# lbrndnr/LBAudioDetective

Measured on AMD Instinct MI355X. Metric: audio_seconds_fingerprinted_per_sec, higher is better.
Workload: dtype f32; 1 GPU; configs[1]: 100k synthetic 1 s @44.1 kHz mono clips, 1024-pt FFT, stride 64, fingerprint-only, input resident in HBM; one step = 13 passes over the batch; clips_per_gpu=100000, samples_per_clip=44100, window=1024, stride=64, bands=32, subfingerprints_per_clip=5, kernel_variant=0, parallelism=clips sharded x1, no collective

## Files before the change

include/lbaudiodetective.h:

```cpp
#ifndef LBAUDIODETECTIVE_H
#define LBAUDIODETECTIVE_H

#include <stddef.h>
#include <stdint.h>

#ifdef __cplusplus
extern "C" {
#endif

#if !defined(__MACTYPES__) && !defined(LBAD_HAVE_MACTYPES)
typedef uint32_t UInt32;
typedef int32_t SInt32;
typedef uint64_t UInt64;
typedef int64_t SInt64;
typedef float Float32;
typedef double Float64;
typedef unsigned char Boolean;
typedef SInt32 OSStatus;
enum { noErr = 0 };
#endif

#if !defined(__CoreAudioTypes_h__) && !defined(LBAD_HAVE_COREAUDIOTYPES)
typedef struct AudioStreamBasicDescription {
    Float64 mSampleRate;
// ... 123 lines not shown

OSStatus LBAudioDetectiveProcessPCM(LBAudioDetectiveRef inDetective, const Float32* inSamples,
                                    UInt64 inNumberOfSamples, LBAudioDetectiveFingerprintRef* outFingerprint);
OSStatus LBAudioDetectiveComparePCM(LBAudioDetectiveRef inDetective, const Float32* inSamples1, UInt64 inCount1,
                                    const Float32* inSamples2, UInt64 inCount2, UInt32 inComparisonRange,
                                    Float32* outMatch);

#define LBAD_PACKED_WORDS 8
#define LBAD_PACKED_BYTES 32
#define LBAD_MAX_SUBFINGERPRINT_LENGTH 256

OSStatus LBAudioDetectiveFingerprintClipsDevice(LBAudioDetectiveRef inDetective, const Float32* inClips,
                                                UInt64 inNumberOfClips, UInt64 inSamplesPerClip,
                                                void* outPacked, void* inStream);
OSStatus LBAudioDetectiveFingerprintClipsDeviceFormat(LBAudioDetectiveRef inDetective, const void* inClips,
                                                      UInt32 inSampleFormat, UInt64 inNumberOfClips,
                                                      UInt64 inSamplesPerClip, void* outPacked, void* inStream);
OSStatus LBAudioDetectiveFingerprintClips(LBAudioDetectiveRef inDetective, const Float32* inClips,
                                          UInt64 inNumberOfClips, UInt64 inSamplesPerClip, Boolean* outBooleans);
OSStatus LBAudioDetectiveFingerprintClipsFormat(LBAudioDetectiveRef inDetective, const void* inClips,
                                                UInt32 inSampleFormat, UInt64 inNumberOfClips,
                                                UInt64 inSamplesPerClip, Boolean* outBooleans);
OSStatus LBAudioDetectiveSetKernelVariant(LBAudioDetectiveRef inDetective, UInt32 inVariant);
OSStatus LBAudioDetectiveSetKernelTuning(LBAudioDetectiveRef inDetective, UInt32 inWavesPerWorkgroup,
                                         UInt32 inTwiddleCache);
OSStatus LBAudioDetectiveSetScratchLimit(LBAudioDetectiveRef inDetective, UInt64 inBytes);
OSStatus LBAudioDetectiveSetStageTiming(LBAudioDetectiveRef inDetective, UInt32 inEnabled);
OSStatus LBAudioDetectiveGetStageTimes(LBAudioDetectiveRef inDetective, Float32* outStage1Ms, Float32* outStage2Ms,
                                       UInt32* outLaunches);
OSStatus LBAudioDetectiveFingerprintClipsDeviceTaps(LBAudioDetectiveRef inDetective, const Float32* inClips,
                                                    UInt64 inNumberOfClips, UInt64 inSamplesPerClip,
                                                    void* outPacked, Float32* outFramesRaw, Float32* outFramesHaar,
                                                    void* inStream);
OSStatus LBAudioDetectiveFingerprintClipsDeviceTapsFormat(LBAudioDetectiveRef inDetective, const void* inClips,
                                                          UInt32 inSampleFormat, UInt64 inNumberOfClips,
                                                          UInt64 inSamplesPerClip, void* outPacked, Float32* outFramesRaw,
                                                          Float32* outFramesHaar, void* inStream);
OSStatus LBAudioDetectiveDebugStage1Choice(Float64 inSampleRate, UInt32 inWindowSize, UInt32 inAnalysisStride,
                                           UInt32 inNumberOfPitchSteps, UInt32 inSubfingerprintLength, UInt32 inKernelVariant,
                                           UInt32 inWavesPerWorkgroup, UInt32 inTwiddleCache, UInt32 inSampleFormat,
                                           UInt64 inNumberOfClips, UInt64 inSamplesPerClip, UInt32 inClipAddressMod8,
                                           UInt32 inRawTap, UInt32 inFileTail, UInt32* outWords, UInt32 inCapacity);

typedef struct LBAudioDetectiveStream* LBAudioDetectiveStreamRef;
LBAudioDetectiveStreamRef LBAudioDetectiveStreamNew(LBAudioDetectiveRef inDetective);
void LBAudioDetectiveStreamDispose(LBAudioDetectiveStreamRef inStream);
// ... 260 lines not shown
```

lbaudiodetective_amd/_native.py:

```python
from __future__ import annotations

import ctypes as C
import os
import subprocess

_HERE = os.path.dirname(os.path.abspath(__file__))
CSRC = os.path.join(_HERE, "csrc")
LIB_PATH = os.path.abspath(os.environ["LBAD_LIB"]) if os.environ.get("LBAD_LIB") else os.path.join(_HERE, "lib", "liblbaudiodetective.so")
HEADER = os.path.join(os.path.dirname(_HERE), "include", "lbaudiodetective.h")

UInt32, SInt32, UInt64, SInt64 = C.c_uint32, C.c_int32, C.c_uint64, C.c_int64
Float32, Float64, Boolean, OSStatus = C.c_float, C.c_double, C.c_ubyte, C.c_int32
Ref = C.c_void_p

PACKED_WORDS = 8
PACKED_BYTES = 32
SHARD_KEYS = 4096
ROWS_PER_FRAME = 128


class AudioStreamBasicDescription(C.Structure):
    _fields_ = [
        ("mSampleRate", Float64), ("mFormatID", UInt32), ("mFormatFlags", UInt32),
        ("mBytesPerPacket", UInt32), ("mFramesPerPacket", UInt32), ("mBytesPerFrame", UInt32),
# ... 67 lines not shown
    "LBAudioDetectiveSetResamplerMode": (OSStatus, [Ref, UInt32]),
    "LBAudioDetectiveReadAudioURLWithResampler": (OSStatus, [C.c_char_p, Float64, UInt32, _P(_P(Float32)), _P(UInt64),
                                                            _P(Float64)]),
    "LBAudioDetectiveProcessFileStream": (OSStatus, [Ref, C.c_void_p, UInt64, UInt64, UInt32, _P(Ref)]),
    "LBAudioDetectiveReadAudioURL": (OSStatus, [C.c_char_p, Float64, _P(_P(Float32)), _P(UInt64), _P(Float64)]),
    "LBAudioDetectiveFreeSamples": (None, [_P(Float32)]),
    "LBAudioDetectiveGetSubfingerprintCount": (UInt64, [Ref, UInt64]),
    "LBAudioDetectiveProcessPCM": (OSStatus, [Ref, C.c_void_p, UInt64, _P(Ref)]),
    "LBAudioDetectiveComparePCM": (OSStatus, [Ref, C.c_void_p, UInt64, C.c_void_p, UInt64, UInt32, _P(Float32)]),
    "LBAudioDetectiveFingerprintClipsDevice": (OSStatus, [Ref, C.c_void_p, UInt64, UInt64, C.c_void_p, C.c_void_p]),
    "LBAudioDetectiveFingerprintClipsDeviceFormat": (OSStatus, [Ref, C.c_void_p, UInt32, UInt64, UInt64, C.c_void_p, C.c_void_p]),
    "LBAudioDetectiveSetFilePipeline": (OSStatus, [Ref, UInt32]),
    "LBAudioDetectiveGetCompactLayout": (OSStatus, [Ref, _P(UInt32), _P(UInt32)]),
    "LBAudioDetectiveGetCompactBands": (OSStatus, [Ref, _P(UInt32), _P(UInt32)]),
    "LBAudioDetectiveCompactFramesToSubfingerprintsDevice": (OSStatus, [Ref, C.c_void_p, UInt64, C.c_void_p, C.c_void_p, C.c_void_p]),
    "LBAudioDetectiveFramesToSubfingerprintsDevice": (OSStatus, [Ref, C.c_void_p, UInt64, C.c_void_p, C.c_void_p, C.c_void_p]),
    "LBAudioDetectiveStreamNew": (Ref, [Ref]),
    "LBAudioDetectiveStreamDispose": (None, [Ref]),
    "LBAudioDetectiveStreamPush": (OSStatus, [Ref, C.c_void_p, UInt64, _P(UInt32)]),
    "LBAudioDetectiveStreamCopyFingerprint": (Ref, [Ref]),
    "LBAudioDetectiveFingerprintClips": (OSStatus, [Ref, C.c_void_p, UInt64, UInt64, C.c_void_p]),
    "LBAudioDetectiveFingerprintClipsFormat": (OSStatus, [Ref, C.c_void_p, UInt32, UInt64, UInt64, C.c_void_p]),
    "LBAudioDetectiveSetKernelVariant": (OSStatus, [Ref, UInt32]),
    "LBAudioDetectiveSetScratchLimit": (OSStatus, [Ref, UInt64]),
    "LBAudioDetectiveSetStageTiming": (OSStatus, [Ref, UInt32]),
    "LBAudioDetectiveGetStageTimes": (OSStatus, [Ref, _P(Float32), _P(Float32), _P(UInt32)]),
    "LBAudioDetectiveFingerprintClipsDeviceTapsFormat": (OSStatus, [Ref, C.c_void_p, UInt32, UInt64, UInt64, C.c_void_p, C.c_void_p,
                                                                    C.c_void_p, C.c_void_p]),
    "LBAudioDetectiveDebugStage1Choice": (OSStatus, [Float64, UInt32, UInt32, UInt32, UInt32, UInt32, UInt32, UInt32, UInt32, UInt64,
                                                     UInt64, UInt32, UInt32, UInt32, _P(UInt32), UInt32]),
    "LBAudioDetectiveFingerprintClipsDeviceTaps": (OSStatus, [Ref, C.c_void_p, UInt64, UInt64, C.c_void_p, C.c_void_p,
                                                              C.c_void_p, C.c_void_p]),
    "LBAudioDetectivePackSubfingerprint": (None, [C.c_void_p, UInt32, C.c_void_p]),
    "LBAudioDetectiveUnpackSubfingerprint": (None, [C.c_void_p, UInt32, C.c_void_p]),
    "LBAudioDetectiveCorpusNew": (Ref, [UInt32, UInt32, UInt64]),
    "LBAudioDetectiveCorpusNewRagged": (Ref, [UInt32, UInt64, UInt64]),
    "LBAudioDetectiveCorpusAppendRaggedPackedDevice": (OSStatus, [Ref, C.c_void_p, C.c_void_p, UInt64, C.c_void_p]),
    "LBAudioDetectiveCorpusGetSubfingerprintTotal": (UInt64, [Ref]),
    "LBAudioDetectiveSynthRaggedCorpusDevice": (OSStatus, [UInt32, UInt64, UInt64, C.c_void_p, UInt64, UInt32, C.c_void_p,
                                                           C.c_void_p]),
    "LBAudioDetectiveCorpusQuerySharded": (OSStatus, [Ref, Ref, UInt32, UInt64, C.c_void_p, C.c_void_p, _P(SInt64), _P(Float32)]),
    "LBAudioDetectiveCorpusQueryBatchSharded": (OSStatus, [Ref, _P(Ref), UInt32, UInt32, UInt64, C.c_void_p, C.c_void_p,
                                                           _P(SInt64), _P(Float32)]),
    "LBAudioDetectiveCorpusQueryBatchShardedWith": (OSStatus, [Ref, _P(Ref), UInt32, UInt32, UInt64, C.c_void_p, C.c_void_p,
                                                               C.c_void_p, _P(SInt64), _P(Float32)]),
    "LBAudioDetectiveSetExchangeTimeout": (None, [UInt32]),
# ... 145 lines not shown
```

lbaudiodetective_amd/api.py:

```python
from __future__ import annotations

import collections
import ctypes as C

import numpy as np

from . import _native as N

noErr = 0


class LBAudioDetectiveError(RuntimeError):
    def __init__(self, status: int, what: str):
        self.status = status
        code = status & 0xFFFFFFFF
        four = bytes([(code >> s) & 0xFF for s in (24, 16, 8, 0)])
        tag = f"'{four.decode()}'" if all(32 <= b < 127 for b in four) else str(status)
        super().__init__(f"{what}: OSStatus {tag}")


def _check(status: int, what: str):
    if status != noErr:
        raise LBAudioDetectiveError(status, what)

# ... 216 lines not shown

    def set_window_size_status(self, v: int) -> int:
        return self._L.LBAudioDetectiveSetWindowSize(self._ref, int(v))

    def configure(self, sample_rate=None, window=None, stride=None, bands=None, subfp_len=None) -> "Detective":
        if sample_rate is not None:
            self.processing_sample_rate = sample_rate
        if window is not None:
            self.window_size = window
        if stride is not None:
            self.analysis_stride = stride
        if bands is not None:
            self.number_of_pitch_steps = bands
        if subfp_len is not None:
            self.subfingerprint_length = subfp_len
        return self

    def set_file_pipeline(self, enabled: bool):
        _check(self._L.LBAudioDetectiveSetFilePipeline(self._ref, 1 if enabled else 0), "SetFilePipeline")
        return self

    def set_kernel_variant(self, variant: int):
        _check(self._L.LBAudioDetectiveSetKernelVariant(self._ref, variant), "SetKernelVariant")

    def set_scratch_limit(self, n_bytes: int):
        _check(self._L.LBAudioDetectiveSetScratchLimit(self._ref, n_bytes), "SetScratchLimit")

    def set_stage_timing(self, enabled: bool):
        _check(self._L.LBAudioDetectiveSetStageTiming(self._ref, int(enabled)), "SetStageTiming")

    def stage_times(self):
        a, b, n = N.Float32(0), N.Float32(0), N.UInt32(0)
        _check(self._L.LBAudioDetectiveGetStageTimes(self._ref, C.byref(a), C.byref(b), C.byref(n)), "GetStageTimes")
        return float(a.value), float(b.value), int(n.value)

    def subfingerprint_count(self, n_samples: int) -> int:
        return int(self._L.LBAudioDetectiveGetSubfingerprintCount(self._ref, n_samples))

    def set_kernel_tuning(self, waves_per_workgroup: int = 0, twiddle_cache: bool = True):
        _check(self._L.LBAudioDetectiveSetKernelTuning(self._ref, waves_per_workgroup, int(twiddle_cache)), "SetKernelTuning")
        return self

    def set_file_hop_mode(self, mode: int):
        _check(self._L.LBAudioDetectiveSetFileHopMode(self._ref, mode), "SetFileHopMode")
        return self

# ... 1064 lines not shown
```

lbaudiodetective_amd/csrc/api_detective.cpp:

```cpp
#include "internal.hpp"
#include "const_div.hpp"

#include <new>
#include "audiofile.hpp"

#include <cmath>
#include <cstdlib>
#include <cstring>

namespace lbad {

uint64_t subfingerprint_count(uint64_t n_samples, uint32_t window, uint32_t stride) {
    if (stride == 0 || n_samples < window) return 0;
    return ((n_samples - window) / stride) / kRowsPerFrame;
}

static bool valid_window(uint32_t w) { return w >= kMinWindow && w <= kMaxWindow && (w & (w - 1)) == 0; }

static void free_plan(Plan& p) { p = Plan(); }

static void plan_kernels_host(Plan& p) {
    p.pruned_ok = rows_pruned_supported(p);
    p.full_ok = rows_full_supported(p);
    p.stream_ok = rows_stream_supported(p);
    p.stream2_ok = rows_stream2_supported(p);
}

static OSStatus plan_kernels_device(Plan& p) {
    if (p.pruned_ok && !p.d_bin_const) {
        std::vector<float> bc;
        rows_pruned_constants(bc);
        OSStatus st = p.d_bin_const.reserve(bc.size());
        if (st != noErr) return st;
        LBAD_HIP(hipMemcpy(p.d_bin_const, bc.data(), bc.size() * sizeof(float), hipMemcpyHostToDevice));
    }
    return p.full_ok || p.stream_ok || p.stream2_ok ? p.d_claim.reserve(8) : noErr;
}

OSStatus plan_host(Plan& p, double rate, uint32_t window, uint32_t stride, uint32_t bands, uint32_t subfp_len) {
    if (!valid_window(window) || stride == 0 || bands == 0 || bands > kMaxBands || !(rate > 0.0) || subfp_len == 0 ||
        subfp_len > LBAD_MAX_SUBFINGERPRINT_LENGTH || subfp_len > kRowsPerFrame * bands)
        return kLBAudioDetectiveArgumentInvalid;
    p.sample_rate = rate;
    p.window = window;
    p.stride = stride;
// ... 41 lines not shown
    LBAD_HIP(hipMemcpy(p.d_tw, re.data(), half * sizeof(float), hipMemcpyHostToDevice));
    LBAD_HIP(hipMemcpy(p.d_tw + half, im.data(), half * sizeof(float), hipMemcpyHostToDevice));
    std::vector<uint32_t> tbl(11 * (size_t)p.bands);
    for (uint32_t b = 0; b < p.bands; ++b) {
        tbl[b] = p.table.lo[b];
        tbl[p.bands + b] = p.table.hi[b];
        const float div = (float)(p.table.indices[b + 1] - p.table.indices[b]);
        std::memcpy(&tbl[2 * p.bands + b], &div, 4);
        tbl[3 * p.bands + b] = p.bands;
        tbl[4 * p.bands + b] = b;
        uint32_t mult = 0, off = 0xFFFFFFFFu;
        if (p.sparse.ok) {
            const uint32_t pos = b >= 16 ? p.sparse.pos_right[b - 16] : (b == p.sparse.left ? p.sparse.pos_left : 0xFFu);
            if (pos != 0xFFu) { mult = p.sparse.n_stored; off = pos; }
        }
        tbl[5 * p.bands + b] = mult;
        tbl[6 * p.bands + b] = off;
        tbl[7 * p.bands + b] = p.table.term_at[b];
        const float rcp = 1.0f / div;
        std::memcpy(&tbl[9 * p.bands + b], &rcp, 4);
        tbl[10 * p.bands + b] = band_div_proven(div) ? 1u : 0u;
    }
    tbl[8 * (size_t)p.bands] = p.table.term_end;
    st = p.d_bands.reserve(tbl.size());
    if (st != noErr) return st;
    LBAD_HIP(hipMemcpy(p.d_bands, tbl.data(), tbl.size() * sizeof(uint32_t), hipMemcpyHostToDevice));
    st = plan_kernels_device(p);
    if (st != noErr) return st;
    p.valid = true;
    return noErr;
}

static hipError_t apply_file_tail(const Plan& p, const FileTail& t, const void* d_pcm, uint64_t rows_total, float* frames,
                                  hipStream_t stream) {
    if (t.mode == 3) return launch_empty_rows_batch(p, t.d_files, t.n_files, t.max_rows, frames, stream);
    const uint64_t rows = t.rows ? t.rows : rows_total;
    if (t.first_short >= rows) return hipSuccess;
    float* file_frames = frames + t.row_begin * p.bands;
    if (t.mode == 1)
        return launch_empty_rows(p, file_frames + t.first_short * p.bands, rows - t.first_short, stream);
    if (t.mode == 2)
        return launch_file_tail(p, static_cast<const float*>(d_pcm) + t.pcm_begin, t.n_client, p.stride, t.first_short,
                                (uint32_t)(rows - t.first_short), t.d_tbl, file_frames, stream);
    return hipSuccess;
}

// ... 80 lines not shown
    }
    w[7] = ch.compact ? 1u : 0u;
    w[8] = ch.stage2_select32 ? (ch.compact ? 2u : 1u) : 0u;
    w[11] = (uint32_t)ch.per;
}

OSStatus fingerprint_clips_device(LBAudioDetective* d, const void* d_pcm_raw, uint32_t fmt, uint64_t n_clips,
                                  uint64_t spc, uint32_t* d_packed, float* d_raw, float* d_haar, hipStream_t stream,
                                  const FileTail* tail, size_t n_tails) {
    if (fmt > 2) return kLBAudioDetectiveArgumentInvalid;
    if (tail && (n_clips != 1 || fmt != 0)) return kLBAudioDetectiveArgumentInvalid;
    LBAD_LOCK(d);
    const size_t elem = fmt == 1 ? 2 : 4;
    const char* d_pcm = static_cast<const char*>(d_pcm_raw);
    OSStatus st = ensure_plan(d);
    if (st != noErr) return st;
    const Plan& p = d->plan;
    Stage1Call call;
    call.variant = d->variant; call.fmt = fmt; call.n_clips = n_clips; call.spc = spc;
    call.ptr_mod8 = (uint32_t)(reinterpret_cast<uintptr_t>(d_pcm_raw) % 8);
    call.raw_tap = d_raw != nullptr; call.tail = tail != nullptr;
    const Stage1Choice ch = stage1_choose(p, call);
    if (ch.status != noErr || !ch.launches) return ch.status;
    const uint64_t per = ch.per;
    StreamOrder order{d, stream};
    LBAD_HIP(order.begin());
    const bool compact = ch.compact;
    auto stage1 = [&](const void* pcm_in, uint64_t nc, float* frames_out) -> hipError_t {
        switch (ch.family) {
            case Stage1Family::Pruned:
                return launch_rows_pruned(p, p.d_bin_const, pcm_in, fmt, nc, spc, (uint32_t)per, frames_out, stream, compact);
            case Stage1Family::Stream2: return launch_rows_stream2(p, pcm_in, fmt, nc, spc, (uint32_t)per, frames_out, stream);
            case Stage1Family::Full: return launch_rows_full(p, pcm_in, fmt, nc, spc, (uint32_t)per, frames_out, stream);
            case Stage1Family::Stream: return launch_rows_stream(p, pcm_in, fmt, nc, spc, (uint32_t)per, frames_out, stream);
            case Stage1Family::Generic: break;
        }
        return launch_fft_bands(p, pcm_in, fmt, nc, spc, (uint32_t)per, frames_out, stream);
    };
    auto stage2 = [&](float* frames_in, uint64_t nf, uint32_t* packed_out, float* haar_out) -> hipError_t {
        if (compact && haar_out) {
            hipError_t e = hipMemsetAsync(haar_out, 0, nf * kRowsPerFrame * p.bands * sizeof(float), stream);
            if (e != hipSuccess) return e;
        }
        return ch.stage2_select32 ? launch_haar_select32(p, frames_in, nf, packed_out, haar_out, stream, compact)
                                  : launch_haar_select(p, frames_in, nf, packed_out, haar_out, stream);
    };
    const uint64_t frame_floats = (uint64_t)kRowsPerFrame * p.bands;
    if (d_raw) {
        LBAD_HIP(stage1(d_pcm, n_clips, d_raw));
        for (size_t t = 0; tail && t < n_tails; ++t) LBAD_HIP(apply_file_tail(p, tail[t], d_pcm, per * kRowsPerFrame, d_raw, stream));
        LBAD_HIP(stage2(d_raw, n_clips * per, d_packed, d_haar));
        return noErr;
    }
    uint64_t chunk = (d->scratch_limit / sizeof(float)) / (per * frame_floats);
// ... 225 lines not shown
    LBAD_LOCK(d);
    d->subfp_len = inSubfingerprintLength;
    return noErr;
}
OSStatus LBAudioDetectiveSetWindowSize(LBAudioDetectiveRef d, UInt32 inWindowSize) {
    LBAD_LOCK(d);
    if (!lbad::valid_window(inWindowSize)) return kLBAudioDetectiveArgumentInvalid;
    d->window = inWindowSize;
    return noErr;
}
OSStatus LBAudioDetectiveSetAnalysisStride(LBAudioDetectiveRef d, UInt32 inAnalysisStride) {
    LBAD_LOCK(d);
    d->stride = inAnalysisStride;
    return noErr;
}

OSStatus LBAudioDetectiveSetKernelVariant(LBAudioDetectiveRef d, UInt32 inVariant) {
    LBAD_LOCK(d);
    if (inVariant > 4) return kLBAudioDetectiveArgumentInvalid;
    d->variant = inVariant;
    return noErr;
}

OSStatus LBAudioDetectiveSetKernelTuning(LBAudioDetectiveRef d, UInt32 inWavesPerWorkgroup, UInt32 inTwiddleCache) {
    LBAD_LOCK(d);
    if (!d || inWavesPerWorkgroup > 16) return kLBAudioDetectiveArgumentInvalid;
    d->tune_waves = inWavesPerWorkgroup;
    d->tune_cache = inTwiddleCache != 0;
    return noErr;
}

OSStatus LBAudioDetectiveSetScratchLimit(LBAudioDetectiveRef d, UInt64 inBytes) {
    LBAD_LOCK(d);
    if (!d || inBytes == 0) return kLBAudioDetectiveArgumentInvalid;
    d->scratch_limit = inBytes;
    return noErr;
}

OSStatus LBAudioDetectiveSetStageTiming(LBAudioDetectiveRef d, UInt32 inEnabled) {
    LBAD_LOCK(d);
    if (!d) return kLBAudioDetectiveArgumentInvalid;
    d->timing = inEnabled != 0;
    d->ev_used = 0;
    return noErr;
}

// ... 511 lines not shown
```

lbaudiodetective_amd/csrc/internal.hpp:

```cpp
#pragma once

#include <hip/hip_runtime.h>

#include <algorithm>
#include <cstdint>
#include <cstdio>
#include <new>
#include <stdexcept>
#include <map>
#include <mutex>
#include <vector>

#include "../../include/lbaudiodetective.h"
#include "buffers.hpp"

namespace lbad {

constexpr uint32_t kRowsPerFrame = 128;
constexpr uint32_t kPackedWords = LBAD_PACKED_WORDS;
constexpr uint32_t kMaxBands = 64;
constexpr uint32_t kSparseFrameDwMax = 128 * 17;
constexpr uint32_t kMinWindow = 16;
constexpr uint32_t kMaxWindow = 8192;

// ... 23 lines not shown
    std::vector<uint32_t> lo, hi;
    uint32_t kmin = 0, kmax = 0;
    std::vector<uint32_t> term_at;
    uint32_t term_end = 0;
    bool ordered = true;
    uint64_t unread_terms16 = 0;
};

void make_band_table(double sample_rate, uint32_t window, uint32_t bands, BandTable& out);
void make_band_bounds(double sample_rate, uint32_t window, uint32_t n_frames, const BandTable& table, uint32_t* lo,
                      uint32_t* hi);
void make_twiddles(uint32_t W, std::vector<float>& re, std::vector<float>& im);

struct Plan {
    double sample_rate = 0;
    uint32_t window = 0, stride = 0, bands = 0, subfp_len = 0;
    uint32_t log2w = 0;
    uint32_t keep = 0;
    BandTable table;
    DeviceBuffer<float> d_tw;
    DeviceBuffer<uint32_t> d_bands;
    DeviceBuffer<float> d_bin_const;
    bool pruned_ok = false;
    bool full_ok = false;
    bool stream_ok = false;
    bool stream2_ok = false;
    DeviceBuffer<uint32_t> d_claim;
    struct Sparse {
        bool ok = false;
        uint32_t left = 32;
        uint32_t n_cols = 0;
        uint8_t cols[32] = {};
        uint32_t n_stored = 0;
        uint8_t stored[17] = {};
        uint8_t pos_right[16];
        uint8_t pos_left = 0xFF;
        uint32_t frame_dw() const { return 128u * n_stored; }
    } sparse;
    uint32_t tune_waves = 0;
    bool tune_cache = true;
    bool valid = false;
};

struct FileDesc;
struct FileTail {
    uint32_t mode = 0;
    const FileDesc* d_files = nullptr;
    uint32_t n_files = 0;
    uint64_t max_rows = 0;
    uint64_t first_short = 0;
    uint64_t n_client = 0;
    const uint32_t* d_tbl = nullptr;
    uint64_t row_begin = 0;
    uint64_t rows = 0;
    uint64_t pcm_begin = 0;
};

hipError_t launch_fft_bands(const Plan& plan, const void* d_pcm, uint32_t fmt, uint64_t n_clips,
                            uint64_t samples_per_clip, uint32_t frames_per_clip, float* d_frames, hipStream_t stream);
hipError_t launch_haar_select(const Plan& plan, float* d_frames, uint64_t n_frames, uint32_t* d_packed,
                              float* d_haar_out, hipStream_t stream);
bool rows_pruned_supported(const Plan& plan);
void rows_pruned_constants(std::vector<float>& out);
hipError_t launch_rows_pruned(const Plan& plan, const float* d_bin_const, const void* d_pcm, uint32_t fmt,
                              uint64_t n_clips, uint64_t samples_per_clip, uint32_t frames_per_clip, float* d_frames,
                              hipStream_t stream, bool compact = false);

bool rows_full_supported(const Plan& plan);
bool rows_full_supported_fmt(const Plan& plan, uint32_t fmt);
hipError_t launch_rows_full(const Plan& plan, const void* d_pcm, uint32_t fmt, uint64_t n_clips,
                            uint64_t samples_per_clip, uint32_t frames_per_clip, float* d_frames, hipStream_t stream);

bool rows_stream_supported(const Plan& plan);
hipError_t launch_rows_stream(const Plan& plan, const void* d_pcm, uint32_t fmt, uint64_t n_clips,
                              uint64_t samples_per_clip, uint32_t frames_per_clip, float* d_frames, hipStream_t stream);

bool rows_stream2_supported(const Plan& plan);
hipError_t launch_rows_stream2(const Plan& plan, const void* d_pcm, uint32_t fmt, uint64_t n_clips,
                               uint64_t samples_per_clip, uint32_t frames_per_clip, float* d_frames, hipStream_t stream);

bool haar_select32_supported(const Plan& plan);
hipError_t launch_haar_select32(const Plan& plan, const float* d_frames, uint64_t n_frames, uint32_t* d_packed,
                                float* d_haar_out, hipStream_t stream, bool compact = false);
void plan_sparse(Plan& plan);

enum class Stage1Family : uint32_t { Generic = 0, Pruned = 1, Stream2 = 2, Full = 3, Stream = 4 };
struct FftBandsInstance {
    uint32_t log2w = 0, wpb = 0;
    bool cached = false;
// ... 353 lines not shown

}

struct LBAudioDetectiveFingerprint {
    uint32_t length = 0;
    uint32_t count = 0;
    std::vector<Boolean> data;
};

struct LBAudioDetectiveFrame {
    uint32_t max_rows = 0;
    uint32_t n_rows = 0;
    uint32_t row_length = 0;
    std::vector<std::vector<Float32>> rows;
};

struct LBAudioDetective {
    AudioStreamBasicDescription format;
    uint32_t subfp_len;
    uint32_t window;
    uint32_t stride;
    uint32_t bands;
    uint32_t variant = 0;
    uint32_t tune_waves = 0;
    bool tune_cache = true;
    uint32_t hop_mode = 1;
    uint32_t tail_mode = 1;
    uint32_t resampler = 0;
    lbad::Plan plan;
    lbad::DeviceBuffer<float> d_frames;
    uint64_t scratch_limit = 512ull << 20;
    lbad::DeviceBuffer<void> d_io_pcm;
    lbad::DeviceBuffer<uint32_t> d_io_packed;
    lbad::PinnedBuffer<void> h_io;
    hipStream_t io_stream = nullptr;
    lbad::DeviceBuffer<uint8_t> d_rs_bytes[2];
    hipStream_t up_stream = nullptr;
    hipEvent_t up_done[2] = {nullptr, nullptr};
    hipEvent_t bytes_free[2] = {nullptr, nullptr};
    hipEvent_t packed_done[2] = {nullptr, nullptr};
    lbad::DeviceBuffer<float> d_rs_in;
    lbad::DeviceBuffer<float> d_rs_out;
    lbad::DeviceBuffer<double> d_rs_table[2];
    std::vector<lbad::DevPhase> d_phases;
    lbad::DeviceBuffer<lbad::FileDesc> d_rs_desc;
    lbad::DeviceBuffer<uint32_t> d_rs_tail;
// ... 82 lines not shown
```

lbaudiodetective_amd/csrc/k_rows_pruned.hip:

```cpp
#include "internal.hpp"
#include "const_div.hpp"
#include "fft64_lane.hpp"

namespace lbad {
namespace {

constexpr int kW = 1024;
constexpr int kStride = 64;
constexpr int kBands = 32;
constexpr int kBins = 22;
constexpr int kRows = 43;
constexpr int kRowsA = 22;
constexpr int kRowDw = 20;
constexpr int kWinDw = 464;
constexpr int kWaves = 4;
constexpr int kThreads = kWaves * 64;
constexpr int kUnitWindows = 32;
constexpr int kSpan = (kUnitWindows - 1) * kStride + kW;
constexpr int kSpanDw = kSpan + 16 * (kSpan >> 6);
constexpr int kTDw = kWaves * 8 * kWinDw;
constexpr int kBinConst = 14;
constexpr int kConstStride = 20;
constexpr int kConstDw = kBins * kConstStride;
constexpr int kClaimOffset = 312;
// ... 319 lines not shown
#ifdef LBAD_EXP_TIMELINE
        STAMP(6);
        if (lane == 0) {
            float* o = frames + ((unit >> 2) * 128 + quarter * kUnitWindows + 8 * wave) * kBands;
            for (int i = 1; i < 7; ++i) o[i - 1] = (float)(ts[i] - ts[i - 1]);
            o[6] = (float)(ts[0] & 0xFFFFFF);
            o[7] = (float)__builtin_amdgcn_s_getreg(((16 - 1) << 11) | 4);
            o[8] = (float)(ts[0] >> 24 & 0xFFFFFF);
            o[9] = (float)(__builtin_amdgcn_s_memrealtime() - rt0);
        }
#endif
        if (next >= xcd_end) break;
        unit = next;
    }
#ifndef LBAD_EXP_TIMELINE
    if (out_ptr) {
#pragma unroll
        for (int q = 0; q < 4; ++q) out_ptr[q * 2 * b_mult] = out[q];
    }
#endif
    if (claimer) claims_done(claim_ctr);
}

}

bool rows_pruned_supported(const Plan& p) {
    if (p.window != (uint32_t)kW || p.stride != (uint32_t)kStride || p.bands != (uint32_t)kBands) return false;
    if (p.table.kmax > (uint32_t)kBins) return false;
    std::vector<float> re, im;
    make_twiddles(kW, re, im);
    for (int t = 0; t < 32; ++t)
        if (re[16 * t] != kTw64Re[t] || im[16 * t] != kTw64Im[t]) return false;
    return true;
}

void rows_pruned_constants(std::vector<float>& out) {
    std::vector<float> re, im;
    make_twiddles(kW, re, im);
    out.assign((size_t)kClaimOffset + kClaimWords, 0.0f);
    for (int k = 0; k < kBins; ++k) {
        float* c = &out[(size_t)k * kBinConst];
        c[0] = re[8 * k]; c[1] = im[8 * k];
        c[2] = re[4 * k]; c[3] = im[4 * k];
        c[4] = re[2 * k]; c[5] = im[2 * k];
        if (k > 0) {
            c[6] = -re[8 * (64 - k)];   c[7] = -im[8 * (64 - k)];
            c[8] = -re[4 * (128 - k)];  c[9] = -im[4 * (128 - k)];
            c[10] = -re[2 * (256 - k)]; c[11] = -im[2 * (256 - k)];
            c[12] = re[k]; c[13] = im[k];
        }
    }
}

template <int FMT>
static hipError_t launch_rows_fmt(const Plan& plan, const float* d_bin_const, const void* d_pcm, uint64_t n_frames,
                                  uint64_t samples_per_clip, uint32_t frames_per_clip, float* d_frames,
                                  hipStream_t stream, bool compact) {
    static PerDevice attr;
    if (attr.changed(kLdsBytes)) {
        hipError_t e = hipFuncSetAttribute(reinterpret_cast<const void*>(frame_rows_pruned_kernel<FMT>),
                                           hipFuncAttributeMaxDynamicSharedMemorySize, kLdsBytes);
        if (e != hipSuccess) return e;
    }
    const uint64_t n_units = n_frames * 4, units_per_xcd = 4 * ((n_frames + 7) / 8);
    const int n_cu = device_cu_count();
    uint64_t wg_per_xcd = ((uint64_t)n_cu * kWgPerCu + 7) / 8;
    if (wg_per_xcd > units_per_xcd / 4) wg_per_xcd = units_per_xcd / 4;
    uint32_t* claim = reinterpret_cast<uint32_t*>(const_cast<float*>(d_bin_const)) + kClaimOffset;
    hipLaunchKernelGGL(frame_rows_pruned_kernel<FMT>, dim3((uint32_t)(wg_per_xcd * 8)), dim3(kThreads), kLdsBytes,
                       stream, d_pcm, samples_per_clip, frames_per_clip, n_units, units_per_xcd, d_bin_const,
                       plan.d_bands, claim, d_frames, compact ? plan.sparse.frame_dw() : 128u * kBands, compact ? 5u : 3u);
    return hipGetLastError();
}

hipError_t launch_rows_pruned(const Plan& plan, const float* d_bin_const, const void* d_pcm, uint32_t fmt,
                              uint64_t n_clips, uint64_t samples_per_clip, uint32_t frames_per_clip, float* d_frames,
                              hipStream_t stream, bool compact) {
    if (compact && !plan.sparse.ok) return hipErrorInvalidValue;
    const uint64_t n_frames = n_clips * frames_per_clip;
    if (n_frames == 0) return hipSuccess;
    if (n_frames > 0x7fffffffull) return hipErrorInvalidValue;
    if (n_frames * 4 + 8 > 0x7fffffffull) return hipErrorInvalidValue;
    switch (fmt) {
        case 0: return launch_rows_fmt<0>(plan, d_bin_const, d_pcm, n_frames, samples_per_clip, frames_per_clip, d_frames, stream, compact);
        case 1: return launch_rows_fmt<1>(plan, d_bin_const, d_pcm, n_frames, samples_per_clip, frames_per_clip, d_frames, stream, compact);
        case 2: return launch_rows_fmt<2>(plan, d_bin_const, d_pcm, n_frames, samples_per_clip, frames_per_clip, d_frames, stream, compact);
        default: return hipErrorInvalidValue;
    }
}

}
```

Before: 5.509 million audio-s/s.

## Add lane-mapped band-sum pruned FFT kernel, selected by default

```diff
diff --git a/include/lbaudiodetective.h b/include/lbaudiodetective.h
--- a/include/lbaudiodetective.h
+++ b/include/lbaudiodetective.h
@@ -169,6 +169,8 @@
                                                 UInt32 inSampleFormat, UInt64 inNumberOfClips,
                                                 UInt64 inSamplesPerClip, Boolean* outBooleans);
 OSStatus LBAudioDetectiveSetKernelVariant(LBAudioDetectiveRef inDetective, UInt32 inVariant);
+OSStatus LBAudioDetectiveSetBandSumForm(LBAudioDetectiveRef inDetective, UInt32 inForm);
+OSStatus LBAudioDetectiveGetBandSumForm(LBAudioDetectiveRef inDetective, UInt32* outForm);
 OSStatus LBAudioDetectiveSetKernelTuning(LBAudioDetectiveRef inDetective, UInt32 inWavesPerWorkgroup,
                                          UInt32 inTwiddleCache);
 OSStatus LBAudioDetectiveSetScratchLimit(LBAudioDetectiveRef inDetective, UInt64 inBytes);
diff --git a/lbaudiodetective_amd/_native.py b/lbaudiodetective_amd/_native.py
--- a/lbaudiodetective_amd/_native.py
+++ b/lbaudiodetective_amd/_native.py
@@ -113,6 +113,8 @@
     "LBAudioDetectiveFingerprintClips": (OSStatus, [Ref, C.c_void_p, UInt64, UInt64, C.c_void_p]),
     "LBAudioDetectiveFingerprintClipsFormat": (OSStatus, [Ref, C.c_void_p, UInt32, UInt64, UInt64, C.c_void_p]),
     "LBAudioDetectiveSetKernelVariant": (OSStatus, [Ref, UInt32]),
+    "LBAudioDetectiveSetBandSumForm": (OSStatus, [Ref, UInt32]),
+    "LBAudioDetectiveGetBandSumForm": (OSStatus, [Ref, _P(UInt32)]),
     "LBAudioDetectiveSetScratchLimit": (OSStatus, [Ref, UInt64]),
     "LBAudioDetectiveSetStageTiming": (OSStatus, [Ref, UInt32]),
     "LBAudioDetectiveGetStageTimes": (OSStatus, [Ref, _P(Float32), _P(Float32), _P(UInt32)]),
diff --git a/lbaudiodetective_amd/api.py b/lbaudiodetective_amd/api.py
--- a/lbaudiodetective_amd/api.py
+++ b/lbaudiodetective_amd/api.py
@@ -262,6 +262,14 @@
 
     def set_kernel_variant(self, variant: int):
         _check(self._L.LBAudioDetectiveSetKernelVariant(self._ref, variant), "SetKernelVariant")
+
+    def set_band_sum_form(self, form: int):
+        _check(self._L.LBAudioDetectiveSetBandSumForm(self._ref, form), "SetBandSumForm")
+
+    def band_sum_form(self) -> int:
+        form = N.UInt32(0)
+        _check(self._L.LBAudioDetectiveGetBandSumForm(self._ref, C.byref(form)), "GetBandSumForm")
+        return int(form.value)
 
     def set_scratch_limit(self, n_bytes: int):
         _check(self._L.LBAudioDetectiveSetScratchLimit(self._ref, n_bytes), "SetScratchLimit")
diff --git a/lbaudiodetective_amd/csrc/api_detective.cpp b/lbaudiodetective_amd/csrc/api_detective.cpp
--- a/lbaudiodetective_amd/csrc/api_detective.cpp
+++ b/lbaudiodetective_amd/csrc/api_detective.cpp
@@ -21,6 +21,7 @@
 
 static void plan_kernels_host(Plan& p) {
     p.pruned_ok = rows_pruned_supported(p);
+    p.lanes_ok = p.pruned_ok && rows_lanes_supported(p);
     p.full_ok = rows_full_supported(p);
     p.stream_ok = rows_stream_supported(p);
     p.stream2_ok = rows_stream2_supported(p);
@@ -108,6 +109,7 @@
         tbl[10 * p.bands + b] = band_div_proven(div) ? 1u : 0u;
     }
     tbl[8 * (size_t)p.bands] = p.table.term_end;
+    rows_lanes_table(p, tbl);
     st = p.d_bands.reserve(tbl.size());
     if (st != noErr) return st;
     LBAD_HIP(hipMemcpy(p.d_bands, tbl.data(), tbl.size() * sizeof(uint32_t), hipMemcpyHostToDevice));
@@ -234,6 +236,7 @@
     call.raw_tap = d_raw != nullptr; call.tail = tail != nullptr;
     const Stage1Choice ch = stage1_choose(p, call);
     if (ch.status != noErr || !ch.launches) return ch.status;
+    if (d->band_form == 2 && !p.lanes_ok) return kLBAudioDetectiveArgumentInvalid;
     const uint64_t per = ch.per;
     StreamOrder order{d, stream};
     LBAD_HIP(order.begin());
@@ -241,7 +244,8 @@
     auto stage1 = [&](const void* pcm_in, uint64_t nc, float* frames_out) -> hipError_t {
         switch (ch.family) {
             case Stage1Family::Pruned:
-                return launch_rows_pruned(p, p.d_bin_const, pcm_in, fmt, nc, spc, (uint32_t)per, frames_out, stream, compact);
+                return launch_rows_pruned(p, p.d_bin_const, pcm_in, fmt, nc, spc, (uint32_t)per, frames_out, stream, compact,
+                                          d->band_form);
             case Stage1Family::Stream2: return launch_rows_stream2(p, pcm_in, fmt, nc, spc, (uint32_t)per, frames_out, stream);
             case Stage1Family::Full: return launch_rows_full(p, pcm_in, fmt, nc, spc, (uint32_t)per, frames_out, stream);
             case Stage1Family::Stream: return launch_rows_stream(p, pcm_in, fmt, nc, spc, (uint32_t)per, frames_out, stream);
@@ -513,6 +517,30 @@
     return noErr;
 }
 
+static bool band_lanes_now(LBAudioDetectiveRef d) {
+    lbad::Plan p;
+    return lbad::plan_host(p, d->format.mSampleRate, d->window, d->stride, d->bands, d->subfp_len) == noErr && p.lanes_ok;
+}
+
+OSStatus LBAudioDetectiveSetBandSumForm(LBAudioDetectiveRef d, UInt32 inForm) {
+    LBAD_GUARD_BEGIN
+    LBAD_LOCK(d);
+    if (!d || inForm > 2) return kLBAudioDetectiveArgumentInvalid;
+    if (inForm == 2 && !band_lanes_now(d)) return kLBAudioDetectiveArgumentInvalid;
+    d->band_form = inForm;
+    return noErr;
+    LBAD_GUARD_END
+}
+
+OSStatus LBAudioDetectiveGetBandSumForm(LBAudioDetectiveRef d, UInt32* outForm) {
+    LBAD_GUARD_BEGIN
+    LBAD_LOCK(d);
+    if (!d || !outForm) return kLBAudioDetectiveArgumentInvalid;
+    *outForm = d->band_form != 1 && band_lanes_now(d) ? 2u : 1u;
+    return noErr;
+    LBAD_GUARD_END
+}
+
 OSStatus LBAudioDetectiveSetKernelTuning(LBAudioDetectiveRef d, UInt32 inWavesPerWorkgroup, UInt32 inTwiddleCache) {
     LBAD_LOCK(d);
     if (!d || inWavesPerWorkgroup > 16) return kLBAudioDetectiveArgumentInvalid;
diff --git a/lbaudiodetective_amd/csrc/internal.hpp b/lbaudiodetective_amd/csrc/internal.hpp
--- a/lbaudiodetective_amd/csrc/internal.hpp
+++ b/lbaudiodetective_amd/csrc/internal.hpp
@@ -69,6 +69,7 @@
     DeviceBuffer<uint32_t> d_bands;
     DeviceBuffer<float> d_bin_const;
     bool pruned_ok = false;
+    bool lanes_ok = false;
     bool full_ok = false;
     bool stream_ok = false;
     bool stream2_ok = false;
@@ -111,7 +112,9 @@
 void rows_pruned_constants(std::vector<float>& out);
 hipError_t launch_rows_pruned(const Plan& plan, const float* d_bin_const, const void* d_pcm, uint32_t fmt,
                               uint64_t n_clips, uint64_t samples_per_clip, uint32_t frames_per_clip, float* d_frames,
-                              hipStream_t stream, bool compact = false);
+                              hipStream_t stream, bool compact = false, uint32_t band_form = 0);
+bool rows_lanes_supported(const Plan& plan);
+void rows_lanes_table(const Plan& plan, std::vector<uint32_t>& band_tbl);
 
 bool rows_full_supported(const Plan& plan);
 bool rows_full_supported_fmt(const Plan& plan, uint32_t fmt);
@@ -511,6 +514,7 @@
     uint32_t stride;
     uint32_t bands;
     uint32_t variant = 0;
+    uint32_t band_form = 0;
     uint32_t tune_waves = 0;
     bool tune_cache = true;
     uint32_t hop_mode = 1;
diff --git a/lbaudiodetective_amd/csrc/k_rows_pruned.hip b/lbaudiodetective_amd/csrc/k_rows_pruned.hip
--- a/lbaudiodetective_amd/csrc/k_rows_pruned.hip
+++ b/lbaudiodetective_amd/csrc/k_rows_pruned.hip
@@ -1,4 +1,6 @@
 #include "internal.hpp"
+
+#include <cstring>
 #include "const_div.hpp"
 #include "fft64_lane.hpp"
 
@@ -365,6 +367,288 @@
     if (claimer) claims_done(claim_ctr);
 }
 
+constexpr int kLaneBands = 15;
+constexpr int kLaneBandLo[kLaneBands] = {0, 1, 2, 3, 4, 5, 6, 7, 8, 9, 11, 12, 14, 17, 19};
+constexpr int kLaneBandHi[kLaneBands] = {1, 2, 3, 4, 5, 6, 7, 8, 9, 11, 12, 14, 17, 19, 22};
+constexpr int kLaneBin[8][3] = {{0, 1, 2}, {3, 4, 5}, {6, 7, 8}, {9, 10, 11}, {14, 15, 16}, {19, 20, 21}, {12, 13, -1}, {17, 18, -1}};
+constexpr int kLanesFirstRow = 11;
+
+constexpr int lanes_pos(int k) {
+    for (int j = 0; j < 8; ++j)
+        for (int rd = 0; rd < 3; ++rd)
+            if (kLaneBin[j][rd] == k) return 8 * rd + j;
+    return -1;
+}
+constexpr int lanes_band_of(int k) {
+    for (int b = 0; b < kLaneBands; ++b)
+        if (k >= kLaneBandLo[b] && k < kLaneBandHi[b]) return b;
+    return -1;
+}
+constexpr uint32_t lanes_cont_mask(int rd) {
+    uint32_t m = 0;
+    for (int j = 0; j < 8; ++j)
+        if (kLaneBin[j][rd] >= 0 && kLaneBin[j][rd] == kLaneBin[j][rd - 1] + 1 &&
+            lanes_band_of(kLaneBin[j][rd]) == lanes_band_of(kLaneBin[j][rd - 1]))
+            m |= 1u << j;
+    return m;
+}
+constexpr uint64_t lanes_bin_pack(int rd) {
+    uint64_t v = 0;
+    for (int j = 0; j < 8; ++j) v |= (uint64_t)(kLaneBin[j][rd] >= 0 ? kLaneBin[j][rd] : 0) << (5 * j);
+    return v;
+}
+constexpr bool lanes_table_ok() {
+    for (int k = 0; k < kBins; ++k)
+        if (lanes_pos(k) < 0 || lanes_pos(k) >= kBins || lanes_band_of(k) < 0) return false;
+    for (int b = 0; b < kLaneBands; ++b) {
+        for (int k = kLaneBandLo[b] + 1; k < kLaneBandHi[b]; ++k)
+            if (lanes_pos(k) != lanes_pos(k - 1) + 8) return false;
+    }
+    return lanes_pos(kBins - 1) == kBins - 1;
+}
+static_assert(lanes_table_ok(), "every bin has one position below 22 and every band lies in one lane, in bin order");
+
+template <int I, int END>
+__device__ __forceinline__ void store_rows_lanes(const cplx (&x)[64], float* trow) {
+    if constexpr (I < END) {
+        *(lds_vf32x2*)(trow + lanes_pos(I) * kRowDw) = stage6_row<I>(x);
+        store_rows_lanes<I + 1, END>(x, trow);
+    }
+}
+template <int I, int N>
+__device__ __forceinline__ void store_held_lanes(const cplx (&h)[kRows - kRowsA], float* trow) {
+    if constexpr (I < N) {
+        *(lds_vf32x2*)(trow + lanes_pos(kBins - 1 - I) * kRowDw) = h[I];
+        store_held_lanes<I + 1, N>(h, trow);
+    }
+}
+
+template <int FMT>
+__global__ __launch_bounds__(kThreads, kWgPerCu) void frame_rows_lanes_kernel(const void* __restrict__ pcm_raw,
+                                                                        uint64_t samples_per_clip,
+                                                                        uint32_t frames_per_clip, uint64_t n_units,
+                                                                        uint64_t units_per_xcd,
+                                                                        const float* __restrict__ bin_const,
+                                                                        const uint32_t* __restrict__ band_tbl,
+                                                                        uint32_t* __restrict__ claim_ctr,
+                                                                        float* __restrict__ frames, uint32_t frame_dw,
+                                                                        uint32_t row_dw, uint32_t place_row) {
+    extern __shared__ __attribute__((aligned(16))) float smem[];
+    float* span = smem;
+    const int wave = __builtin_amdgcn_readfirstlane(threadIdx.x >> 6);
+    const int lane = threadIdx.x & 63;
+    float* tbuf = smem + kSpanDw + wave * (8 * kWinDw);
+    float* cbuf = smem + kSpanDw + kTDw;
+    static_assert((kSpanDw + kTDw + kConstDw) % 2 == 0, "the slot behind the constants is 8-byte aligned");
+    typedef __attribute__((address_space(3))) volatile uint64_t lds_vu64;
+    lds_vu64* next_slot = (lds_vu64*)(cbuf + kConstDw);
+
+    const uint32_t wg_per_xcd = gridDim.x >> 3;
+    const uint64_t xcd_begin = (uint64_t)(blockIdx.x & 7) * units_per_xcd;
+    const uint64_t xcd_end = xcd_begin + units_per_xcd < n_units ? xcd_begin + units_per_xcd : n_units;
+    uint64_t unit = xcd_begin + 4 * (uint64_t)(blockIdx.x >> 3);
+    if (unit >= xcd_end) {
+        if (threadIdx.x == 0) claims_done(claim_ctr);
+        return;
+    }
+
+    auto span_start = [&](uint64_t u) {
+        const uint32_t frame = (uint32_t)(u >> 2);
+        const uint32_t clip = frame / frames_per_clip;
+        const uint32_t fi = frame - clip * frames_per_clip;
+        return (uint64_t)clip * samples_per_clip + (uint64_t)(fi * 128 + (uint32_t)(u & 3) * kUnitWindows) * kStride;
+    };
+    uint32_t* my_ctr = claim_ctr + (blockIdx.x & 7);
+    asm volatile("" : "+v"(my_ctr));
+    const bool claimer = threadIdx.x == 0;
+    uint32_t claimed = 0;
+    uint64_t claim_base = xcd_begin + 4 * (uint64_t)wg_per_xcd;
+    asm volatile("" : "+s"(claim_base));
+
+    span_to_lds<FMT>(pcm_raw, span_start(unit), span, wave, lane);
+    for (int i = threadIdx.x; i < kBins * kBinConst; i += kThreads) {
+        const int p = i / kBinConst;
+        constexpr uint64_t kBin0 = lanes_bin_pack(0), kBin1 = lanes_bin_pack(1), kBin2 = lanes_bin_pack(2);
+        const int k = (int)(((p < 8 ? kBin0 : p < 16 ? kBin1 : kBin2) >> (5 * (p & 7))) & 31u);
+        cbuf[p * kConstStride + (i % kBinConst)] = bin_const[k * kBinConst + (i % kBinConst)];
+    }
+
+    const int w8 = lane >> 3, r = lane & 7;
+    const float inv_norm = 1.0f / (float)(kW / 4);
+    const int rr = r ^ ((((w8 + 1) >> 1) & 1) << 2);
+    int tk[3];
+#pragma unroll
+    for (int rd = 0; rd < 3; ++rd) tk[rd] = rr + 8 * rd < kBins ? rr + 8 * rd : kBins - 1;
+
+    const uint32_t* task_tbl = band_tbl + kLanesFirstRow * kBands;
+    float t_div[3], t_rcp[3];
+    uint32_t t_off = 0, z_off = 0;
+    bool proven = true;
+#pragma unroll
+    for (int rd = 0; rd < 3; ++rd) {
+        t_div[rd] = __uint_as_float(task_tbl[8 * rd + rr]);
+        t_rcp[rd] = __uint_as_float(task_tbl[kBands + 8 * rd + rr]);
+        proven = proven && task_tbl[2 * kBands + 8 * rd + rr] != 0u;
+        t_off |= (task_tbl[place_row * kBands + 8 * rd + rr] & 0xFFu) << (8 * rd);
+        z_off |= (task_tbl[5 * kBands + 8 * rd + rr] & 0xFFu) << (8 * rd);
+    }
+    const int t_fast_hi = proven ? (int)kBandDivHi : -1;
+    constexpr uint32_t kCont1 = lanes_cont_mask(1), kCont2 = lanes_cont_mask(2);
+    const uint32_t m_cont1 = (kCont1 >> rr) & 1u ? 0xFFFFFFFFu : 0u;
+    const uint32_t m_cont2 = (kCont2 >> rr) & 1u ? 0xFFFFFFFFu : 0u;
+    const bool is_dc = rr == 0;
+
+    __syncthreads();
+    TreeTw twp[3], twm[3];
+    f32x2 ws[3];
+#pragma unroll
+    for (int rd = 0; rd < 3; ++rd) {
+        const float* c = cbuf + tk[rd] * kConstStride;
+        twp[rd] = tree_twiddles(c);
+        twm[rd] = tree_twiddles(c + 6);
+        ws[rd] = *reinterpret_cast<const f32x2*>(c + 12);
+    }
+
+    float out[3] = {0.0f, 0.0f, 0.0f};
+    float* out_row = nullptr;
+#ifdef LBAD_EXP_TIMELINE
+    long long ts[8];
+#define STAMP(i) ts[i] = __builtin_readcyclecounter()
+#else
+#define STAMP(i)
+#endif
+    auto store_out = [&]() {
+        if (!out_row) return;
+        uint32_t places = t_off;
+        asm volatile("" : "+v"(places));
+#pragma unroll
+        for (int rd = 0; rd < 3; ++rd) {
+            const uint32_t o = (places >> (8 * rd)) & 0xFFu;
+            if (o != 0xFFu) out_row[o] = out[rd];
+        }
+        uint32_t layout = place_row;
+        asm volatile("" : "+s"(layout));
+        if (layout == 3u) {
+            places = z_off;
+            asm volatile("" : "+v"(places));
+#pragma unroll
+            for (int rd = 0; rd < 3; ++rd) {
+                const uint32_t o = (places >> (8 * rd)) & 0xFFu;
+                if (o != 0xFFu) out_row[o] = 0.0f;
+            }
+        }
+    };
+    for (;;) {
+        STAMP(0);
+#ifdef LBAD_EXP_TIMELINE
+        const unsigned long long rt0 = __builtin_amdgcn_s_memrealtime();
+#endif
+        __builtin_amdgcn_s_waitcnt(0x0F70);
+        const uint32_t quarter = (uint32_t)(unit & 3);
+        if (quarter == 3 && claimer) *next_slot = claim_base + 4 * (uint64_t)claimed;
+        __syncthreads();
+        STAMP(1);
+
+        cplx x[64];
+        load_points<0>(x, span + 80 * (8 * wave + w8) + 2 * r);
+        const uint64_t next = quarter == 3 ? *next_slot : unit + 1;
+        __syncthreads();
+        if (next < xcd_end) span_to_lds<FMT>(pcm_raw, span_start(next), span, wave, lane);
+        if (quarter == 0 && claimer) claimed = atomicAdd(my_ctr, 1u);
+#ifndef LBAD_EXP_TIMELINE
+        store_out();
+#endif
+        STAMP(2);
+
+        __builtin_amdgcn_s_setprio(0);
+        stage_blocks<1, 0>(x);
+        stage_blocks<2, 0>(x);
+        stage_blocks<3, 0>(x);
+        stage_blocks<4, 0>(x);
+        stage_blocks<5, 0>(x);
+        STAMP(3);
+        __builtin_amdgcn_s_setprio(3);
+
+        store_rows_lanes<0, kRowsA>(x, tbuf + w8 * kWinDw + 2 * r);
+        cplx held[kRows - kRowsA];
+        hold_rows<kRowsA, kRows, kRowsA>(x, held);
+        cplx za[3];
+        {
+            TreeIn in[3];
+#pragma unroll
+            for (int rd = 0; rd < 3; ++rd) in[rd] = tree_load(tbuf + w8 * kWinDw + tk[rd] * kRowDw);
+            store_held_lanes<0, kRows - kRowsA>(held, tbuf + w8 * kWinDw + 2 * r);
+#pragma unroll
+            for (int rd = 0; rd < 3; ++rd) za[rd] = tree_eval(in[rd], twp[rd]);
+        }
+        STAMP(4);
+        float pw[3];
+        {
+            TreeIn in[3];
+#pragma unroll
+            for (int rd = 0; rd < 3; ++rd) in[rd] = tree_load(tbuf + w8 * kWinDw + tk[rd] * kRowDw);
+#pragma unroll
+            for (int rd = 0; rd < 3; ++rd) {
+                const cplx b = tree_eval(in[rd], twm[rd]);
+                const cplx a = za[rd];
+                float re, im;
+                if (rd == 0 && is_dc) {
+                    const float sm = a.x + a.y, df = a.x - a.y;
+                    re = sm + sm;
+                    im = df + df;
+                } else {
+                    const float sr = a.x + b.x, si = a.y - b.y;
+                    const float dr = a.x - b.x, di = a.y + b.y;
+                    const float wr = ws[rd].x, wi = ws[rd].y;
+                    re = __fmaf_rn(wr, di, __fmaf_rn(wi, dr, sr));
+                    im = __fmaf_rn(-wr, dr, __fmaf_rn(wi, di, si));
+                }
+                if (re > 0.0f) re = __fmul_rn(re, inv_norm);
+                if (im > 0.0f) im = __fmul_rn(im, inv_norm);
+                pw[rd] = __fadd_rn(__fmul_rn(re, re), __fmul_rn(im, im));
+            }
+        }
+        STAMP(5);
+
+        float s[3];
+#pragma unroll
+        for (int rd = 0; rd < 3; ++rd) s[rd] = pw[rd] < INFINITY ? pw[rd] : 0.0f;
+        s[1] = __fadd_rn(__uint_as_float(__float_as_uint(s[0]) & m_cont1), s[1]);
+        s[2] = __fadd_rn(__uint_as_float(__float_as_uint(s[1]) & m_cont2), s[2]);
+        DivGuard g;
+        g.dividends(s[0], s[1]);
+        g.dividends(s[2], s[2]);
+        const int s_max = max(max((int)__float_as_uint(s[0]), (int)__float_as_uint(s[1])), (int)__float_as_uint(s[2]));
+        if (__builtin_expect(__builtin_amdgcn_ballot_w64(g.lo < 2u * kBandDivLo - 1u || s_max > t_fast_hi) == 0, 1)) {
+#pragma unroll
+            for (int rd = 0; rd < 3; ++rd) out[rd] = div_c<true>(s[rd], t_div[rd], t_rcp[rd]);
+        } else {
+#pragma unroll
+            for (int rd = 0; rd < 3; ++rd) out[rd] = div_c<false>(s[rd], t_div[rd], t_rcp[rd]);
+        }
+        out_row = frames + (unit >> 2) * frame_dw + (quarter * kUnitWindows + 8 * wave + w8) * row_dw;
+#ifdef LBAD_EXP_TIMELINE
+        asm volatile("" ::"v"(out[0]), "v"(out[1]), "v"(out[2]));
+        STAMP(6);
+        if (lane == 0) {
+            float* o = frames + ((unit >> 2) * 128 + quarter * kUnitWindows + 8 * wave) * kBands;
+            for (int i = 1; i < 7; ++i) o[i - 1] = (float)(ts[i] - ts[i - 1]);
+            o[6] = (float)(ts[0] & 0xFFFFFF);
+            o[7] = (float)__builtin_amdgcn_s_getreg(((16 - 1) << 11) | 4);
+            o[8] = (float)(ts[0] >> 24 & 0xFFFFFF);
+            o[9] = (float)(__builtin_amdgcn_s_memrealtime() - rt0);
+        }
+#endif
+        if (next >= xcd_end) break;
+        unit = next;
+    }
+#ifndef LBAD_EXP_TIMELINE
+    store_out();
+#endif
+    if (claimer) claims_done(claim_ctr);
+}
+#undef STAMP
+
 }
 
 bool rows_pruned_supported(const Plan& p) {
@@ -395,13 +679,71 @@
     }
 }
 
+static bool lanes_bands_match(const Plan& p) {
+    if (p.window != (uint32_t)kW || p.bands != (uint32_t)kBands || p.table.lo.size() != (size_t)kBands ||
+        p.table.indices.size() != (size_t)kBands + 1)
+        return false;
+    int n = 0;
+    for (int b = 0; b < kBands; ++b) {
+        if (p.table.lo[b] >= p.table.hi[b]) {
+            if (p.table.indices[b + 1] == p.table.indices[b]) return false;
+            continue;
+        }
+        if (n == kLaneBands || p.table.lo[b] != (uint32_t)kLaneBandLo[n] || p.table.hi[b] != (uint32_t)kLaneBandHi[n]) return false;
+        ++n;
+    }
+    return n == kLaneBands;
+}
+
+bool rows_lanes_supported(const Plan& p) { return rows_pruned_supported(p) && lanes_bands_match(p); }
+
+void rows_lanes_table(const Plan& p, std::vector<uint32_t>& tbl) {
+    if (!lanes_bands_match(p)) return;
+    tbl.resize((size_t)(kLanesFirstRow + 6) * kBands, 0u);
+    uint32_t* t = &tbl[(size_t)kLanesFirstRow * kBands];
+    const float one = 1.0f;
+    for (int i = 0; i < kBands; ++i) {
+        std::memcpy(&t[i], &one, 4);
+        std::memcpy(&t[kBands + i], &one, 4);
+        t[2 * kBands + i] = 1u;
+        t[3 * kBands + i] = t[4 * kBands + i] = t[5 * kBands + i] = 0xFFFFFFFFu;
+    }
+    int empty = 0;
+    for (uint32_t b = 0; b < (uint32_t)kBands; ++b) {
+        if (p.table.lo[b] >= p.table.hi[b]) {
+            if (empty < 24) t[5 * kBands + empty] = b;
+            ++empty;
+            continue;
+        }
+        const float div = (float)(p.table.indices[b + 1] - p.table.indices[b]);
+        const float rcp = 1.0f / div;
+        for (uint32_t k = p.table.lo[b]; k < p.table.hi[b]; ++k) {
+            const int at = lanes_pos((int)k);
+            std::memcpy(&t[at], &div, 4);
+            std::memcpy(&t[kBands + at], &rcp, 4);
+            t[2 * kBands + at] = band_div_proven(div) ? 1u : 0u;
+            if (k + 1 != p.table.hi[b]) continue;
+            t[3 * kBands + at] = b;
+            if (p.sparse.ok) {
+                const uint32_t pos = b >= 16 ? p.sparse.pos_right[b - 16] : (b == p.sparse.left ? p.sparse.pos_left : 0xFFu);
+                if (pos != 0xFFu) t[4 * kBands + at] = pos;
+            }
+        }
+    }
+}
+
 template <int FMT>
 static hipError_t launch_rows_fmt(const Plan& plan, const float* d_bin_const, const void* d_pcm, uint64_t n_frames,
                                   uint64_t samples_per_clip, uint32_t frames_per_clip, float* d_frames,
-                                  hipStream_t stream, bool compact) {
-    static PerDevice attr;
-    if (attr.changed(kLdsBytes)) {
+                                  hipStream_t stream, bool compact, bool lanes) {
+    static PerDevice attr, attr_lanes;
+    if (!lanes && attr.changed(kLdsBytes)) {
         hipError_t e = hipFuncSetAttribute(reinterpret_cast<const void*>(frame_rows_pruned_kernel<FMT>),
+                                           hipFuncAttributeMaxDynamicSharedMemorySize, kLdsBytes);
+        if (e != hipSuccess) return e;
+    }
+    if (lanes && attr_lanes.changed(kLdsBytes)) {
+        hipError_t e = hipFuncSetAttribute(reinterpret_cast<const void*>(frame_rows_lanes_kernel<FMT>),
                                            hipFuncAttributeMaxDynamicSharedMemorySize, kLdsBytes);
         if (e != hipSuccess) return e;
     }
@@ -410,24 +752,32 @@
     uint64_t wg_per_xcd = ((uint64_t)n_cu * kWgPerCu + 7) / 8;
     if (wg_per_xcd > units_per_xcd / 4) wg_per_xcd = units_per_xcd / 4;
     uint32_t* claim = reinterpret_cast<uint32_t*>(const_cast<float*>(d_bin_const)) + kClaimOffset;
-    hipLaunchKernelGGL(frame_rows_pruned_kernel<FMT>, dim3((uint32_t)(wg_per_xcd * 8)), dim3(kThreads), kLdsBytes,
-                       stream, d_pcm, samples_per_clip, frames_per_clip, n_units, units_per_xcd, d_bin_const,
-                       plan.d_bands, claim, d_frames, compact ? plan.sparse.frame_dw() : 128u * kBands, compact ? 5u : 3u);
+    if (lanes)
+        hipLaunchKernelGGL(frame_rows_lanes_kernel<FMT>, dim3((uint32_t)(wg_per_xcd * 8)), dim3(kThreads), kLdsBytes,
+                           stream, d_pcm, samples_per_clip, frames_per_clip, n_units, units_per_xcd, d_bin_const,
+                           plan.d_bands, claim, d_frames, compact ? plan.sparse.frame_dw() : 128u * kBands,
+                           compact ? plan.sparse.n_stored : (uint32_t)kBands, compact ? 4u : 3u);
+    else
+        hipLaunchKernelGGL(frame_rows_pruned_kernel<FMT>, dim3((uint32_t)(wg_per_xcd * 8)), dim3(kThreads), kLdsBytes,
+                           stream, d_pcm, samples_per_clip, frames_per_clip, n_units, units_per_xcd, d_bin_const,
+                           plan.d_bands, claim, d_frames, compact ? plan.sparse.frame_dw() : 128u * kBands, compact ? 5u : 3u);
     return hipGetLastError();
 }
 
 hipError_t launch_rows_pruned(const Plan& plan, const float* d_bin_const, const void* d_pcm, uint32_t fmt,
                               uint64_t n_clips, uint64_t samples_per_clip, uint32_t frames_per_clip, float* d_frames,
-                              hipStream_t stream, bool compact) {
+                              hipStream_t stream, bool compact, uint32_t band_form) {
     if (compact && !plan.sparse.ok) return hipErrorInvalidValue;
+    if (band_form > 2 || (band_form == 2 && !plan.lanes_ok)) return hipErrorInvalidValue;
+    const bool lanes = band_form != 1 && plan.lanes_ok;
     const uint64_t n_frames = n_clips * frames_per_clip;
     if (n_frames == 0) return hipSuccess;
     if (n_frames > 0x7fffffffull) return hipErrorInvalidValue;
     if (n_frames * 4 + 8 > 0x7fffffffull) return hipErrorInvalidValue;
     switch (fmt) {
-        case 0: return launch_rows_fmt<0>(plan, d_bin_const, d_pcm, n_frames, samples_per_clip, frames_per_clip, d_frames, stream, compact);
-        case 1: return launch_rows_fmt<1>(plan, d_bin_const, d_pcm, n_frames, samples_per_clip, frames_per_clip, d_frames, stream, compact);
-        case 2: return launch_rows_fmt<2>(plan, d_bin_const, d_pcm, n_frames, samples_per_clip, frames_per_clip, d_frames, stream, compact);
+        case 0: return launch_rows_fmt<0>(plan, d_bin_const, d_pcm, n_frames, samples_per_clip, frames_per_clip, d_frames, stream, compact, lanes);
+        case 1: return launch_rows_fmt<1>(plan, d_bin_const, d_pcm, n_frames, samples_per_clip, frames_per_clip, d_frames, stream, compact, lanes);
+        case 2: return launch_rows_fmt<2>(plan, d_bin_const, d_pcm, n_frames, samples_per_clip, frames_per_clip, d_frames, stream, compact, lanes);
         default: return hipErrorInvalidValue;
     }
 }
```

After: 5.706 million audio-s/s, median of 6. +3.6%, better.
